# liuhx02/YourEditableAvatar

Hardware: AMD Instinct MI355X
Metric: rasterized fragments/sec (fwd+bwd) @500k Gaussians 1080p (higher is better)
Workload: dtype f32

## Files before the change

youreditableavatar_amd/csrc/tgs_api.hip:

```cpp
#include "tgs_device.hpp"
#include "../../include/tgs_raster.h"
#include "../../include/tgs_raster_testing.h"

#include <cstdarg>
#include <cstdio>
#include <cstring>

namespace tgs {
void launch_preprocess_fwd(hipStream_t, const FwdIn&, const CamParams&, const GeomState&, const ImgState&);
void launch_preprocess_fwd_batch(hipStream_t, const FwdIn&, const FwdViews&);
void launch_scan(hipStream_t, const GeomState&, const ImgState&, uint32_t nblocks, uint32_t T, uint32_t sort_cap, unsigned long long r_capacity,
                 uint32_t tile_bound, uint32_t heavy_bound, uint32_t mid_bound, Meta* host_meta, int light);
void launch_bin_count(hipStream_t, int P, const GeomState&, const ImgState&, uint32_t gx, uint32_t T);
void launch_scatter(hipStream_t, int P, const GeomState&, const ImgState&, const BinState&, uint32_t gx, uint32_t T);
void launch_tile_sort(hipStream_t, const GeomState&, const ImgState&, const BinState&, uint32_t gx, uint32_t T, uint64_t r_bound, const Meta* m,
                      uint32_t sort_cap, uint32_t tile_bound, uint32_t heavy_bound, uint32_t mid_bound);
void launch_render_fwd(hipStream_t, const ImgState&, const BinState&, int W, int H, uint32_t gx, uint32_t T, const Meta* m, const float* bg,
                       float* out_color, uint32_t tile_bound, uint32_t mid_bound, int light);
void launch_mark_visible(hipStream_t, int P, const float* means3D, const float* view, uint8_t* present);
void launch_render_bwd(hipStream_t, const ImgState&, const BinState&, int W, int H, uint32_t gx, uint32_t tiles, const float* bg, const float* dL_dpix,
                       bool deterministic, uint32_t mid_tiles, int light, uint32_t T);
void launch_preprocess_bwd(hipStream_t, const BwdIn&, const CamParams&, const GeomState&, const BinState&);
void launch_preprocess_bwd_batch(hipStream_t, const BwdIn&, const BatchViews&);
void launch_selftest_reduce36(hipStream_t, const float* in, float* out);
// ... 771 lines not shown

int tgs_backward_batch_range(void* stream, int P, int D, int M, int n_views, const tgs_view_t* views, const float* means3D, const float* shs,
                             const float* scales, float scale_modifier, const float* rotations, const float* cov3D_precomp, float* dL_dopacity,
                             float* dL_dmean3D, float* dL_dcov3D, float* dL_dsh, float* dL_dscale, float* dL_drot, int accumulate, int first, int count)
{
    return tgs_backward_batch_range_planes(stream, P, D, M, n_views, views, means3D, shs, scales, scale_modifier, rotations, cov3D_precomp, dL_dopacity, dL_dmean3D,
                                           dL_dcov3D, dL_dsh, dL_dscale, dL_drot, accumulate, first, count, 0);
}

int tgs_backward_batch_range_planes(void* stream, int P, int D, int M, int n_views, const tgs_view_t* views, const float* means3D, const float* shs,
                                    const float* scales, float scale_modifier, const float* rotations, const float* cov3D_precomp, float* dL_dopacity,
                                    float* dL_dmean3D, float* dL_dcov3D, float* dL_dsh, float* dL_dscale, float* dL_drot, int accumulate, int first, int count,
                                    int64_t dsh_plane_stride)
{
    hipStream_t st = (hipStream_t)stream;
    g_err[0] = 0;
    if (P == 0 || n_views == 0 || count == 0) return TGS_OK;
    if (P < 0 || n_views < 0 || !views) return fail(TGS_ERR_INVALID, "bad sizes");
    if (first < 0 || count < 0 || first % PRE_BLOCK != 0 || (long long)first + count > P || ((first + count) % PRE_BLOCK != 0 && first + count != P))
        return fail(TGS_ERR_INVALID, "Gaussian range [%d, %d + %d) must start and end on multiples of %d (or end at P = %d)", first, first, count, PRE_BLOCK, P);
    const Model m{P, D, M, means3D, shs, nullptr, nullptr, scales, scale_modifier, rotations, cov3D_precomp};
    const bool has_sh = m.has_sh(), has_sr = m.has_sr();
    if (int r = check_model(m, MODEL_BATCH_BACKWARD)) return r;
    if (!dL_dopacity || !dL_dmean3D || (has_sh && !dL_dsh) || (has_sr && (!dL_dscale || !dL_drot)) || (!has_sr && !dL_dcov3D))
        return fail(TGS_ERR_INVALID, "NULL required pointer");
    if (dsh_plane_stride != 0 && (!has_sh || M != 16 || dsh_plane_stride < 3 * (int64_t)P || dsh_plane_stride % 4 != 0 || ((uintptr_t)dL_dsh & 15u) != 0))
        return fail(TGS_ERR_INVALID, "level-major dL_dsh needs SH colours with M = 16, a plane stride >= 3 P that is a multiple of 4 floats, and a 16-byte aligned dL_dsh");
    BwdIn in = bwd_in(m);
    in.dL_dopacity = dL_dopacity; in.dL_dmean3D = dL_dmean3D; in.dL_dcov3D = has_sr ? nullptr : dL_dcov3D; in.dL_dsh = dL_dsh;
    in.dL_dscale = has_sr ? dL_dscale : nullptr; in.dL_drot = has_sr ? dL_drot : nullptr;
    in.block0 = first / PRE_BLOCK; in.nblocks = (int)n_blocks((size_t)count);
    in.dsh_plane = (long long)dsh_plane_stride;
    for (int v0 = 0; v0 < n_views; v0 += BATCH_VIEWS) {
        BatchViews bv;
        memset(&bv, 0, sizeof(bv));
        bv.n = n_views - v0 < BATCH_VIEWS ? n_views - v0 : BATCH_VIEWS;
        for (int k = 0; k < bv.n; k++) {
            const tgs_view_t& w = views[v0 + k];
            if (int r = check_view(w, v0 + k, VIEW_BATCH_BWD, has_sh)) return r;
            const ViewArgs v = view_args(w);
            const FrameBuffers fb = carve_frame(m.shape(), v, w.R, w.geom_buffer, w.binning_buffer, w.img_buffer);
            BatchView& o = bv.v[k];
            o.cam = v.cam(scale_modifier); o.g = fb.g; o.b = fb.b;
            o.meta = fb.s.meta; o.radii = w.radii; o.dL_dmean2D = w.dL_dmean2D; o.dL_dcolor = has_sh ? nullptr : w.dL_dcolor;
        }
        in.accumulate = (accumulate || v0 > 0) ? 1 : 0;
        if (int r = stage(st, TGS_STAGE_PREPROCESS_BWD, "preprocess_bwd_batch", 0, [&] { launch_preprocess_bwd_batch(st, in, bv); })) return r;
    }
    return TGS_OK;
}

int tgs_mark_visible(void* stream, int P, const float* means3D, const float* viewmatrix, const float* projmatrix, uint8_t* present)
{
    hipStream_t st = (hipStream_t)stream;
    g_err[0] = 0;
    (void)projmatrix;
    if (P == 0) return TGS_OK;
    if (P < 0 || !means3D || !viewmatrix || !present) return fail(TGS_ERR_INVALID, "bad arguments");
    launch_mark_visible(st, P, means3D, viewmatrix, present);
    hipError_t e = hipGetLastError();
    if (e != hipSuccess) return fail(TGS_ERR_HIP, "mark_visible: %s", hipGetErrorString(e));
    return TGS_OK;
}

int64_t tgs_state_field(void* stream, const char* field, int P, int width, int height, int64_t R, int has_sh, int has_scale_rot,
                        const void* geom_buffer, const void* binning_buffer, const void* img_buffer, void* dst, size_t dst_bytes)
{
    hipStream_t st = (hipStream_t)stream;
    g_err[0] = 0;
    const ViewArgs v{nullptr, width, height, nullptr, nullptr, nullptr, 0.f, 0.f};
    const size_t N = v.N(), T = v.T();
    const FrameBuffers fb = carve_frame(GeomShape{(size_t)P, has_sh != 0, has_scale_rot != 0}, v, R, geom_buffer, binning_buffer, img_buffer);
    const GeomState& g = fb.g; const ImgState& s = fb.s; const BinState& b = fb.b;
    const void* src = nullptr; size_t count = 0, esz = 4, stride = 0, rows = 0;
    if (!strcmp(field, "n_contrib")) { src = s.n_contrib; count = N; }
    else if (!strcmp(field, "final_T")) { src = s.final_T; count = N; }
    else if (!strcmp(field, "ranges")) { src = s.ranges; count = 2 * T; }
    else if (!strcmp(field, "means2D")) { src = g.pack; count = 2 * (size_t)P; esz = 8; stride = 64; rows = (size_t)P; }
    else if (!strcmp(field, "depths")) { src = g.depth; count = (size_t)P; }
    else if (!strcmp(field, "conic_opacity")) { src = (const char*)g.pack + 8; count = 4 * (size_t)P; esz = 16; stride = 64; rows = (size_t)P; }
    else if (!strcmp(field, "rgb")) { src = (const char*)g.pack + 24; count = 3 * (size_t)P; esz = 12; stride = 64; rows = (size_t)P; }
    else if (!strcmp(field, "tiles_touched")) { src = g.tiles_touched; count = (size_t)P; }
    else if (!strcmp(field, "tile_order")) { src = s.tile_order; count = T; }
    else if (!strcmp(field, "stamps")) { src = s.stamps; count = 8 * T; esz = 8; }
    else if (!strcmp(field, "block_masks")) { src = (const char*)b.recC + 4; count = (size_t)R; esz = 4; stride = 8; rows = (size_t)R; }
    else if (!strcmp(field, "quad_masks")) { src = b.qmask; count = (size_t)R; esz = 8; }
    else if (!strcmp(field, "point_list")) { src = b.keys; count = (size_t)R; esz = 4; stride = 8; rows = (size_t)R; }
    else return fail(TGS_ERR_INVALID, "unknown field %s", field);
    const size_t total = stride ? rows * esz : count * esz;
    if (dst_bytes < total) return fail(TGS_ERR_INVALID, "dst too small for %s", field);
    if (count == 0) return 0;
    if (stride) HIP_TRY(hipMemcpy2DAsync(dst, esz, src, stride, esz, rows, hipMemcpyDeviceToDevice, st));
    else HIP_TRY(hipMemcpyAsync(dst, src, total, hipMemcpyDeviceToDevice, st));
    return (int64_t)count;
}

}
```

youreditableavatar_amd/csrc/tgs_forward.hip:

```cpp
#include "tgs_device.hpp"

namespace tgs {

__device__ __forceinline__ float conic_min_on_edge(float dfix, float lo, float hi, float Pfix, float Pvar, float B, float mB_over_Pvar)
{
    const float t = fminf(hi, fmaxf(lo, dfix * mB_over_Pvar));
    return 0.5f * (Pfix * dfix * dfix + Pvar * t * t) + B * dfix * t;
}

__device__ __forceinline__ unsigned long long quadrant_mask(float2 xy, float4 co, uint32_t tx, uint32_t ty)
{
    const float o255 = 255.0f * co.w;
    if (o255 < 0.999f) return 0ull;
    const float tau = (fmaxf(__logf(o255), 0.f) + 0.01f) * 1.001f;
    const float A = co.x, B = co.y, Cc = co.z;
    const float det = A * Cc - B * B;
    if (!(det > 0.f && A > 0.f && Cc > 0.f)) return ~0ull;
    const float rA = __builtin_amdgcn_rcpf(A), K = 2.f * A * tau, sl = -B * rA;
    const float ox = xy.x - (float)(tx * TILE), y0 = (float)(ty * TILE) - xy.y;
    uint32_t keep[2] = {0u, 0u};
#pragma unroll
    for (int R = 0; R < 8; R++) {
        const float dy0 = y0 + (float)(2 * R), dy1 = y0 + (float)(2 * R + 1);
        const float d0 = fmaf(-det * dy0, dy0, K), d1 = fmaf(-det * dy1, dy1, K);
// ... 809 lines not shown
            for (uint32_t i = threadIdx.x; i < n; i += 1024) b.keys[td.y + i] = lk[i];
        }
    } else if (blockIdx.x < heavy_blocks + mid_blocks) {
        const uint32_t grp = threadIdx.x >> 8, tid = threadIdx.x & 255u;
        const uint32_t t = n_heavy + (blockIdx.x - heavy_blocks) * 4 + grp;
        if (n_heavy + (blockIdx.x - heavy_blocks) * 4 >= n_mid) return;
        uint32_t n = 0, start = 0, tile = 0;
        if (t < n_mid) { const uint4 td = s.tile_desc[t]; tile = td.x; start = td.y; n = td.z - td.y; }
        for (uint32_t i = tid; i < n; i += 256) b.tile_of[start + i] = tile;
        if (n > 1024u || n > sort_cap) n = 0;
        unsigned long long* seg = lk + grp * 1024;
        for (uint32_t i = tid; i < n; i += 256) seg[i] = b.keys[start + i];
        if (tid == 0) grp_npad[grp] = n < 2 ? 2u : next_pow2(n);
        __syncthreads();
        const uint32_t npad_wg = max(max(grp_npad[0], grp_npad[1]), max(grp_npad[2], grp_npad[3]));
        sort_tile_lds<256>(seg, tid, n, npad_wg);
        for (uint32_t i = tid; i < n; i += 256) b.keys[start + i] = seg[i];
    } else {
        const uint32_t t = n_mid + (blockIdx.x - heavy_blocks - mid_blocks) * 16 + wv;
        if (t >= n_nonempty) return;
        const uint4 td = s.tile_desc[t];
        const uint32_t n = td.z - td.y;
        for (uint32_t i = lane; i < n; i += 64) b.tile_of[td.y + i] = td.x;
        if (n < 2 || n > sort_cap || n > SORT_CHUNK) return;
        unsigned long long k0, k1;
        regs_load_chunk(b.keys + td.y, 0u, n, lane, k0, k1);
        if (n >= 2) {
            regs_sort128(k0, k1, lane);
            regs_store_chunk(b.keys + td.y, 0u, n, lane, k0, k1);
        }
    }
}

#ifndef TGS_FIN_E
#define TGS_FIN_E 2
#endif
constexpr int FIN_E = TGS_FIN_E;
__global__ __launch_bounds__(256) void k_finalize(const GeomState g, const ImgState s, const BinState b, uint32_t gx, uint32_t T)
{
    if (frame_rejected(s)) return;
    const uint32_t R = (uint32_t)s.meta->R;
    const uint32_t p0 = blockIdx.x * (256 * FIN_E) + threadIdx.x;
    if (p0 >= R) return;
    uint32_t id[FIN_E], tile[FIN_E];
#pragma unroll
    for (int e = 0; e < FIN_E; e++) {
        const uint32_t pc = min(p0 + e * 256, R - 1u);
        id[e] = (uint32_t)b.keys[pc];
        tile[e] = b.tile_of[pc];
    }
    float4 q0[FIN_E], q1[FIN_E], q2[FIN_E], q3[FIN_E];
#pragma unroll
    for (int e = 0; e < FIN_E; e++) {
        const float4* pk = g.pack + 4 * (size_t)id[e];
        q0[e] = pk[0]; q1[e] = pk[1]; q2[e] = pk[2]; q3[e] = pk[3];
    }
#pragma unroll
    for (int e = 0; e < FIN_E; e++) {
        const uint32_t p = p0 + e * 256;
        if (p < R) finalize_entry(q0[e], q1[e], q2[e], q3[e], p, tile[e], gx, b);
    }
}

__device__ __forceinline__ void fill_tile_background(const ImgState& s, uint32_t tile, uint32_t t, int W, int H, uint32_t gx,
                                                     const float* __restrict__ bg, float* __restrict__ out_color)
{
    const int px = (tile % gx) * TILE + (t & 15), py = (tile / gx) * TILE + (t >> 4);
    if (px < W && py < H) {
        const size_t pix_id = (size_t)W * py + px, N = (size_t)W * H;
        s.final_T[pix_id] = 1.0f;
        s.n_contrib[pix_id] = 0;
        out_color[pix_id] = bg[0]; out_color[N + pix_id] = bg[1]; out_color[2 * N + pix_id] = bg[2];
    }
}

constexpr int FQ_THREADS = 256;
#ifndef TGS_FQ_CH
#define TGS_FQ_CH 256
#endif
constexpr int FQ_CH = TGS_FQ_CH;
constexpr int FQ_EPT = FQ_CH / FQ_THREADS;
static_assert(FQ_CH % FQ_THREADS == 0 && FQ_CH >= LIGHT_MAX && FQ_CH <= 768, "whole entries per thread; a light tile is one round; slots are 10-bit in the block lists");
constexpr int FQ_NULL = FQ_CH;

__device__ __forceinline__ bool fwd_q_block_round(const float4* sA, const float4* sB, const float* sC, const uint2* sQ, unsigned short* list,
                                                  unsigned short (*ql)[QL_ROW_F], uint32_t cnt, int blk, int lane, uint32_t cbase, float pixfx, float pixfy,
                                                  float vone, const QuadMasks& qm, bool& done, float& T, float& C0, float& C1, float& C2, uint32_t& last_contributor)
{
    const int qd = lane >> 4, e = lane & 3;
    const uint32_t n = (uint32_t)__builtin_amdgcn_readfirstlane((int)build_own_list_q<FQ_CH>(list, sQ, cnt, blk, lane));
    const unsigned short* myq = &ql[qd][e];
#pragma unroll 1
    for (uint32_t c0 = 0; c0 < n; c0 += QCH_F) {
        const uint32_t nq = (uint32_t)__builtin_amdgcn_readfirstlane((int)build_chunk_quadrant_lists_128(ql, list, c0, n, lane, FQ_NULL));
        uint32_t jn = myq[0];
#pragma unroll 1
        for (uint32_t k = 0; k < nq; k += 4) {
            const uint32_t j = jn;
            jn = myq[k + 4];
            const float4 a = sA[j];
            const float4 bb = sB[j];
            const float cc = sC[j];
            const float dx = a.x - pixfx, dy = a.y - pixfy;
#if TGS_FAST_MATH
            const float power2 = pair_power2(a.z, a.w, bb.x, dx, dy);
            const float alpha = fminf(0.99f, bb.y * __builtin_amdgcn_exp2f(power2));
#else
            const float power2 = -0.5f * (a.z * dx * dx + bb.x * dy * dy) - a.w * dx * dy;
            const float alpha = fminf(0.99f, bb.y * expf(power2));
#endif
            const bool live = !done && !(power2 > 0.0f) && !(alpha < 1.0f / 255.0f);
            const float pown = live ? 1.f - alpha : 1.0f;
            float y, x, x3;
            fwd_chain4(pown, T, y, x, vone, qm);
            const bool fail = live && (x < 0.0001f);
            const bool upd = live && !fail;
            float cand = fail ? y : -1.0f;
            quad_max_bcast3(cand, x, x3);
            const float w = upd ? alpha * y : 0.f;
            C0 += bb.z * w; C1 += bb.w * w; C2 += cc * w;
            last_contributor = upd ? cbase + j : last_contributor;
            const bool stop = cand >= 0.0f;
            T = stop ? cand : x3;
            done = done || stop;
            if (__builtin_amdgcn_ballot_w64(!done) == 0) return true;
        }
    }
    return false;
}

__device__ __forceinline__ uint32_t fwd_q_block_store(const ImgState& s, float* __restrict__ out_color, int W, int H, int px, int py, bool inside, int lane,
                                                      float bg0, float bg1, float bg2, float T, float C0, float C1, float C2, uint32_t last_contributor)
{
    TGS_DPP_ADD(C0, 0xB1, 0xf); TGS_DPP_ADD(C0, 0x4E, 0xf);
    TGS_DPP_ADD(C1, 0xB1, 0xf); TGS_DPP_ADD(C1, 0x4E, 0xf);
    TGS_DPP_ADD(C2, 0xB1, 0xf); TGS_DPP_ADD(C2, 0x4E, 0xf);
    {
        uint32_t o = (uint32_t)__builtin_amdgcn_update_dpp(0, (int)last_contributor, 0xB1, 0xf, 0xf, false);
        last_contributor = max(last_contributor, o);
        o = (uint32_t)__builtin_amdgcn_update_dpp(0, (int)last_contributor, 0x4E, 0xf, 0xf, false);
        last_contributor = max(last_contributor, o);
    }
    if (inside && (lane & 3) == 0) {
        const size_t pix_id = (size_t)W * py + px, N = (size_t)W * H;
        s.final_T[pix_id] = T;
        s.n_contrib[pix_id] = last_contributor;
        out_color[pix_id] = C0 + T * bg0;
        out_color[N + pix_id] = C1 + T * bg1;
        out_color[2 * N + pix_id] = C2 + T * bg2;
    }
    return wave_max_u32(inside ? last_contributor : 0u);
}

__global__ __launch_bounds__(FQ_THREADS, 8) void k_render_fwd(const ImgState s, const BinState b, int W, int H, uint32_t gx,
                                                              const float* __restrict__ bg, float* __restrict__ out_color, uint32_t n_tiles, int light)
{
    __shared__ float4 sA[FQ_CH + 1];
    __shared__ float4 sB[FQ_CH + 1];
    __shared__ float sC[FQ_CH + 1];
    __shared__ uint2 sQ[FQ_CH];
    __shared__ __attribute__((aligned(16))) unsigned short lists[4][FQ_CH + 8];
    __shared__ __attribute__((aligned(16))) unsigned short qlists[4][4][QL_ROW_F];
    __shared__ uint32_t wave_alive[2][4];
    __shared__ uint32_t wave_qmax[4];
    const float bg0 = bg[0], bg1 = bg[1], bg2 = bg[2];
    const uint32_t hk = blockIdx.x >> 3, ht8 = (hk >> 2) * 8u + (blockIdx.x & 7u), quarter = hk & 3u;
    const uint4 tdh = s.tile_desc[min(ht8, n_tiles - 1u)];
    const uint4 ff = frame_counts(s);
    const uint32_t n_all = (ff.x & META_ERR_CAPACITY) ? 0u : ff.y;
    const uint32_t n_ne = light ? min(ff.w, n_all) : n_all;
    const uint32_t n_light = n_all - n_ne;
    const uint32_t heavy_wgs = 4u * ((n_ne + 7u) & ~7u);
    if (blockIdx.x == 0 && threadIdx.x == 0 && heavy_wgs + n_light > gridDim.x) atomicOr(&s.meta->error, META_ERR_TILE_BOUND);
    const int wv = threadIdx.x >> 6, lane = threadIdx.x & 63;
    const int qd = lane >> 4, pq = (lane >> 2) & 3;
    float vone = 1.0f;
    asm volatile("" : "+v"(vone));
    const QuadMasks qm = quad_masks();
    if (threadIdx.x == 0) { sA[FQ_NULL] = make_float4(0.f, 0.f, 0.f, 0.f); sB[FQ_NULL] = make_float4(0.f, 0.f, 0.f, 0.f); sC[FQ_NULL] = 0.f; }

    if (blockIdx.x >= heavy_wgs) {
        const uint32_t li = blockIdx.x - heavy_wgs;
        if (li >= n_light) {
            const uint32_t nfill = gridDim.x - heavy_wgs - n_light, j = li - n_light;
            for (uint32_t i = n_all + j; i < n_tiles; i += nfill)
                fill_tile_background(s, s.tile_desc[i].x, threadIdx.x, W, H, gx, bg, out_color);
            return;
        }
        const uint4 td = s.light_desc[li];
        const uint32_t tile = td.x, n = td.z - td.y;
        const uint32_t tx = tile % gx, ty = tile / gx;
        stamp(s, tile, 0);
        if (threadIdx.x < n) {
            const uint32_t pos = td.y + threadIdx.x;
            float4 va = b.recA[pos], vb = b.recB[pos];
            const float vc = b.recC[pos].x; const uint2 vq = b.qmask[pos];
#if TGS_FAST_MATH
            stage_conic_a(va); stage_conic_b(vb);
#endif
            sA[threadIdx.x] = va; sB[threadIdx.x] = vb; sC[threadIdx.x] = vc; sQ[threadIdx.x] = vq;
        }
        __syncthreads();
        uint32_t wq = 0;
#pragma unroll 1
        for (int bi = 0; bi < 4; bi++) {
            const int bx = (wv + bi) & 3, by = bi, blk = 4 * by + bx;
            const int px = tx * TILE + bx * 4 + (qd & 1) * 2 + (pq & 1);
            const int py = ty * TILE + by * 4 + (qd >> 1) * 2 + (pq >> 1);
            const bool inside = px < W && py < H;
            bool done = !inside;
            if (__builtin_amdgcn_ballot_w64(!done) == 0) continue;
            float T = 1.0f, C0 = 0.f, C1 = 0.f, C2 = 0.f;
            uint32_t last_contributor = 0;
            fwd_q_block_round(sA, sB, sC, sQ, lists[wv], qlists[wv], n, blk, lane, 1u, (float)px, (float)py, vone, qm, done, T, C0, C1, C2, last_contributor);
            wq = max(wq, fwd_q_block_store(s, out_color, W, H, px, py, inside, lane, bg0, bg1, bg2, T, C0, C1, C2, last_contributor));
        }
        if (lane == 0) wave_qmax[wv] = wq;
        __syncthreads();
        if (threadIdx.x == 0) {
            const uint32_t q = max(max(wave_qmax[0], wave_qmax[1]), max(wave_qmax[2], wave_qmax[3]));
            reinterpret_cast<uint32_t*>(&s.light_desc[li])[3] = q;
            reinterpret_cast<uint32_t*>(&s.tile_desc[n_ne + li])[3] = q;
        }
        stamp(s, tile, 1);
        return;
    }
    if (ht8 >= n_ne) return;
    const uint32_t tile = tdh.x;
    const uint32_t tx = tile % gx, ty = tile / gx;
    const int bx = 2 * (int)(quarter & 1u) + (wv & 1), by = 2 * (int)(quarter >> 1) + (wv >> 1), blk = 4 * by + bx;
    const int px = tx * TILE + bx * 4 + (qd & 1) * 2 + (pq & 1);
    const int py = ty * TILE + by * 4 + (qd >> 1) * 2 + (pq >> 1);
    const bool inside = px < W && py < H;
    const float pixfx = (float)px, pixfy = (float)py;
    const uint2 rg = make_uint2(tdh.y, tdh.z);
    set_wave_priority(rg.y - rg.x);
    if (quarter == 0) stamp(s, tile, 0);
    bool done = !inside;
    float T = 1.0f, C0 = 0.f, C1 = 0.f, C2 = 0.f;
    uint32_t last_contributor = 0;
    float4 ra[FQ_EPT], rb[FQ_EPT]; float rc[FQ_EPT]; uint2 rq[FQ_EPT];
#pragma unroll
    for (int i = 0; i < FQ_EPT; i++) { ra[i] = make_float4(0.f, 0.f, 0.f, 0.f); rb[i] = ra[i]; rc[i] = 0.f; rq[i] = make_uint2(0u, 0u); }
#define TGS_FQ_FETCH(BASE) { _Pragma("unroll") for (int i = 0; i < FQ_EPT; i++) { const uint32_t pos = (BASE) + (uint32_t)(i * FQ_THREADS) + threadIdx.x; \
        if (pos < rg.y) { ra[i] = b.recA[pos]; rb[i] = b.recB[pos]; rc[i] = b.recC[pos].x; rq[i] = b.qmask[pos]; } } }
    TGS_FQ_FETCH(rg.x)
    bool wave_live = __builtin_amdgcn_ballot_w64(!done) != 0;
    int round = 0;
    for (uint32_t base = rg.x; base < rg.y; base += FQ_CH, round++) {
        if (lane == 0) wave_alive[round & 1][wv] = wave_live ? 1u : 0u;
        __syncthreads();
        {
            const uint4 f = *reinterpret_cast<const uint4*>(wave_alive[round & 1]);
            if ((f.x | f.y | f.z | f.w) == 0u) break;
        }
        const uint32_t cnt = min((uint32_t)FQ_CH, rg.y - base);
#pragma unroll
        for (int i = 0; i < FQ_EPT; i++) {
            const uint32_t h = (uint32_t)(i * FQ_THREADS) + threadIdx.x;
            if (h < cnt) {
                float4 va = ra[i], vb = rb[i];
#if TGS_FAST_MATH
                stage_conic_a(va); stage_conic_b(vb);
#endif
                sA[h] = va; sB[h] = vb; sC[h] = rc[i]; sQ[h] = rq[i];
            }
        }
        __syncthreads();
        if (base + FQ_CH < rg.y) TGS_FQ_FETCH(base + FQ_CH)
        if (wave_live && fwd_q_block_round(sA, sB, sC, sQ, lists[wv], qlists[wv], cnt, blk, lane, base - rg.x + 1, pixfx, pixfy, vone, qm, done, T, C0, C1, C2, last_contributor))
            wave_live = false;
    }
#undef TGS_FQ_FETCH
    const uint32_t m = fwd_q_block_store(s, out_color, W, H, px, py, inside, lane, bg0, bg1, bg2, T, C0, C1, C2, last_contributor);
    if (lane == 0) wave_qmax[wv] = m;
    __syncthreads();
    if (threadIdx.x == 0) {
        const uint32_t q = max(max(wave_qmax[0], wave_qmax[1]), max(wave_qmax[2], wave_qmax[3]));
        atomicMax(reinterpret_cast<uint32_t*>(&s.tile_desc[ht8]) + 3, q);
        if (ht8 >= ff.w) atomicMax(reinterpret_cast<uint32_t*>(&s.light_desc[ht8 - ff.w]) + 3, q);
    }
    stamp_max(s, tile, 1);
}

__global__ __launch_bounds__(256) void k_mark_visible(int P, const float* __restrict__ means3D, const float* __restrict__ view, uint8_t* present)
{
    const int idx = blockIdx.x * 256 + threadIdx.x;
    if (idx >= P) return;
    const float mx = means3D[3 * (size_t)idx], my = means3D[3 * (size_t)idx + 1], mz = means3D[3 * (size_t)idx + 2];
    const float z = view[2] * mx + view[6] * my + view[10] * mz + view[14];
    present[idx] = !(z <= 0.2f);
}

void launch_preprocess_fwd(hipStream_t st, const FwdIn& in, const CamParams& cam, const GeomState& g, const ImgState& s)
{
    const dim3 grid((unsigned)n_blocks(in.P)), blk(PRE_BLOCK);
    const bool sh = in.colors_precomp == nullptr, sr = in.cov3D_precomp == nullptr;
    FwdView vw;
    vw.cam = cam; vw.g = g; vw.s = s; vw.radii = in.radii;
    if (sh && sr) hipLaunchKernelGGL((k_preprocess_fwd<true, true>), grid, blk, 0, st, in, vw);
    else if (sh) hipLaunchKernelGGL((k_preprocess_fwd<true, false>), grid, blk, 0, st, in, vw);
    else if (sr) hipLaunchKernelGGL((k_preprocess_fwd<false, true>), grid, blk, 0, st, in, vw);
    else hipLaunchKernelGGL((k_preprocess_fwd<false, false>), grid, blk, 0, st, in, vw);
}
void launch_preprocess_fwd_batch(hipStream_t st, const FwdIn& in, const FwdViews& views)
{
    const dim3 grid((unsigned)n_blocks(in.P)), blk(PRE_BLOCK);
    const bool sh = in.colors_precomp == nullptr, sr = in.cov3D_precomp == nullptr;
    if (views.n == 2) {
        if (sh && sr) hipLaunchKernelGGL((k_preprocess_fwd_pair<true, true>), grid, blk, 0, st, in, views.v[0], views.v[1]);
        else if (sh) hipLaunchKernelGGL((k_preprocess_fwd_pair<true, false>), grid, blk, 0, st, in, views.v[0], views.v[1]);
        else if (sr) hipLaunchKernelGGL((k_preprocess_fwd_pair<false, true>), grid, blk, 0, st, in, views.v[0], views.v[1]);
        else hipLaunchKernelGGL((k_preprocess_fwd_pair<false, false>), grid, blk, 0, st, in, views.v[0], views.v[1]);
        return;
    }
    if (sh && sr) hipLaunchKernelGGL((k_preprocess_fwd_batch<true, true>), grid, blk, 0, st, in, views);
    else if (sh) hipLaunchKernelGGL((k_preprocess_fwd_batch<true, false>), grid, blk, 0, st, in, views);
    else if (sr) hipLaunchKernelGGL((k_preprocess_fwd_batch<false, true>), grid, blk, 0, st, in, views);
    else hipLaunchKernelGGL((k_preprocess_fwd_batch<false, false>), grid, blk, 0, st, in, views);
}
void launch_scan(hipStream_t st, const GeomState& g, const ImgState& s, uint32_t nblocks, uint32_t T, uint32_t sort_cap, unsigned long long r_capacity,
                 uint32_t tile_bound, uint32_t heavy_bound, uint32_t mid_bound, Meta* host_meta, int light)
{
    hipLaunchKernelGGL(k_scan, dim3(1u + (T + SCAN_THREADS - 1) / SCAN_THREADS), dim3(SCAN_THREADS), 0, st, g, s, nblocks, T, sort_cap, r_capacity, tile_bound, heavy_bound, mid_bound,
                       host_meta, light);
}
void bin_shape(int P, uint32_t T, uint32_t& nchunks, uint32_t& chunk, uint32_t& band, size_t& lds)
{
    static const int bin_wgs = [] {
        const char* e = getenv("TGS_BIN_WGS");
        const int v = e ? atoi(e) : BIN_WGS_MAX;
        return v < 1 ? 1 : (v > BIN_WGS_MAX ? BIN_WGS_MAX : v);
    }();
    const uint32_t per = ((uint32_t)P + (uint32_t)bin_wgs - 1) / (uint32_t)bin_wgs;
    chunk = (per + BIN_THREADS - 1) / BIN_THREADS * BIN_THREADS;
    if (chunk == 0) chunk = BIN_THREADS;
    nchunks = ((uint32_t)P + chunk - 1) / chunk;
    band = T < BIN_LDS_TILES ? T : BIN_LDS_TILES;
    lds = (size_t)band * sizeof(uint32_t);
}
void launch_bin_count(hipStream_t st, int P, const GeomState& g, const ImgState& s, uint32_t gx, uint32_t T)
{
    uint32_t nchunks, chunk, band; size_t lds;
    bin_shape(P, T, nchunks, chunk, band, lds);
    if (lds > 32 * 1024) (void)hipFuncSetAttribute((const void*)k_bin_count, hipFuncAttributeMaxDynamicSharedMemorySize, (int)lds);
    hipLaunchKernelGGL(k_bin_count, dim3(nchunks), dim3(BIN_THREADS), lds, st, P, chunk, g, s, gx, T, band);
    hipLaunchKernelGGL(k_bin_colscan, dim3((T + WAVE - 1) / WAVE), dim3(64 * COL_WAVES), 0, st, s, T, nchunks);
}
void launch_scatter(hipStream_t st, int P, const GeomState& g, const ImgState& s, const BinState& b, uint32_t gx, uint32_t T)
{
    uint32_t nchunks, chunk, band; size_t lds;
    bin_shape(P, T, nchunks, chunk, band, lds);
    if (lds > 32 * 1024) (void)hipFuncSetAttribute((const void*)k_scatter, hipFuncAttributeMaxDynamicSharedMemorySize, (int)lds);
    hipLaunchKernelGGL(k_scatter, dim3(nchunks), dim3(BIN_THREADS), lds, st, P, chunk, g, s, b, gx, T, band);
}
static uint32_t host_next_pow2(uint32_t n) { uint32_t p = 1; while (p < n) p <<= 1; return p; }
// ... 46 lines not shown
```

youreditableavatar_amd/diff_gaussian_rasterization/_C.py:

```python
from __future__ import annotations

import ctypes as C
import os
from typing import Optional, Tuple

import torch

from .. import build as _build

_LIB_PATH = os.environ.get("TGS_LIBRARY") or _build.LIB


ABI_VERSION = 3


def _load() -> C.CDLL:
    if "TGS_LIBRARY" not in os.environ:
        try:
            _build.build_native()
        except Exception as e:
            what = "is older than its sources" if os.path.exists(_LIB_PATH) else "is missing"
            raise ImportError(f"libtgs_raster.so {what} and could not be rebuilt ({e}); run "
                              f"`python -c 'import __graft_entry__ as g; g.build()'` on a ROCm machine") from e
    lib = C.CDLL(_LIB_PATH, mode=C.RTLD_GLOBAL)
# ... 280 lines not shown
    arr = (C.c_void_p * max(1, len(stream_handles)))(*stream_handles)
    _lib.tgs_set_render_streams(arr, len(stream_handles))


def backward_render_views(stream_handles, P, views, n_views, opt: Optional[_OptionsT] = None) -> None:
    arr = (C.c_void_p * len(stream_handles))(*stream_handles)
    r = _lib.tgs_backward_render_views_opt(C.byref(opt) if opt is not None else None, arr, len(stream_handles), int(P), int(n_views),
                                           views if isinstance(views, C.c_void_p) else C.cast(views, C.c_void_p))
    if r < 0:
        raise _err(int(r))


def backward_batch_raw(stream, P, D, M, views, n_views, means3D, shs, scales, scale_modifier, rotations, dL_dopacity, dL_dmean3D, dL_dsh, dL_dscale,
                       dL_drot, accumulate, first: int = 0, count: Optional[int] = None, dsh_plane_stride: int = 0) -> None:
    args = (stream, int(P), int(D), int(M), int(n_views), views if isinstance(views, C.c_void_p) else C.cast(views, C.c_void_p), means3D, shs,
            scales, float(scale_modifier),
            rotations, None, dL_dopacity, dL_dmean3D, None, dL_dsh if shs else None, dL_dscale, dL_drot, 1 if accumulate else 0,
            int(first), int(P - first if count is None else count))
    r = _lib.tgs_backward_batch_range_planes(*args, int(dsh_plane_stride)) if dsh_plane_stride else _lib.tgs_backward_batch_range(*args)
    if r < 0:
        raise _err(int(r))


def rasterize_gaussians_backward_render(background, dL_dout_color, R, binningBuffer, imageBuffer, P, tile_bound: int = 0,
                                        deterministic: Optional[bool] = None) -> None:
    dev = _require_gpu(dL_dout_color)
    H, W = int(dL_dout_color.size(1)), int(dL_dout_color.size(2))
    with torch.cuda.device(dev):
        bg, dL = _dev_f32(background, dev, "background"), _dev_f32(dL_dout_color, dev, "dL_dout_color")
        opt = options(tile_bound=tile_bound, deterministic=deterministic)
        r = _lib.tgs_backward_render_opt(C.byref(opt), torch.cuda.current_stream(dev).cuda_stream, int(P), int(R), _p(bg), W, H, binningBuffer.data_ptr(),
                                         imageBuffer.data_ptr(), _p(dL))
    if r < 0:
        raise _err(int(r))


def rasterize_gaussians_backward_batch(views, means3D, sh, degree, scales, rotations, scale_modifier, cov3D_precomp, into, accumulate=True):
    dev = _require_gpu(means3D)
    P = int(means3D.size(0))
    M = int(sh.size(1)) if (sh is not None and sh.dim() > 1 and sh.size(0) != 0) else 0
    has_sh = M > 0
    outs = []
    if P == 0 or not views:
        return outs
    with torch.cuda.device(dev):
        t = dict(means=_dev_f32(means3D, dev, "means3D"), sh=_dev_f32(sh, dev, "sh") if has_sh else None, scales=_dev_f32(scales, dev, "scales"),
                 rots=_dev_f32(rotations, dev, "rotations"), cov=_dev_f32(cov3D_precomp, dev, "cov3D_precomp"))
        has_sr = t["scales"] is not None
        arr = (_ViewT * len(views))()
        keep = []
        for i, v in enumerate(views):
            vm, pm, cp = _dev_f32(v["viewmatrix"], dev, "viewmatrix"), _dev_f32(v["projmatrix"], dev, "projmatrix"), _dev_f32(v["campos"], dev, "campos")
            radii = v["radii"].contiguous()
            g2d = torch.empty((P, 3), dtype=torch.float32, device=dev)
            gcol = None if has_sh else torch.empty((P, 3), dtype=torch.float32, device=dev)
            keep += [vm, pm, cp, radii]
            a = arr[i]
            a.width, a.height, a.tan_fovx, a.tan_fovy = int(v["image_width"]), int(v["image_height"]), float(v["tanfovx"]), float(v["tanfovy"])
            a.viewmatrix, a.projmatrix, a.campos, a.radii = vm.data_ptr(), pm.data_ptr(), cp.data_ptr(), radii.data_ptr()
            a.geom_buffer, a.binning_buffer, a.img_buffer, a.R = v["geom"].data_ptr(), v["binning"].data_ptr(), v["img"].data_ptr(), int(v["R"])
            a.dL_dmean2D, a.dL_dcolor = g2d.data_ptr(), (gcol.data_ptr() if gcol is not None else None)
            outs.append((g2d, gcol))

        def dst(name, shape):
            g = into.get(name)
            if g is None:
                raise RuntimeError(f"rasterize_gaussians_backward_batch: no gradient buffer for {name}")
            if g.dtype != torch.float32 or g.device != dev or not g.is_contiguous() or tuple(g.shape) != shape:
                raise RuntimeError(f"gradient buffer for {name} must be a contiguous fp32 tensor of shape {shape} on {dev}")
            return g.data_ptr()

        r = _lib.tgs_backward_batch(torch.cuda.current_stream(dev).cuda_stream, P, int(degree), M, len(views), C.cast(arr, C.c_void_p), _p(t["means"]),
                                    _p(t["sh"]), _p(t["scales"]), float(scale_modifier), _p(t["rots"]), _p(t["cov"]), dst("opacities", (P, 1)),
                                    dst("means3D", (P, 3)), None if has_sr else dst("cov3D_precomp", (P, 6)), dst("sh", (P, M, 3)) if has_sh else None,
                                    dst("scales", (P, 3)) if has_sr else None, dst("rotations", (P, 4)) if has_sr else None, 1 if accumulate else 0)
        del keep
    if r < 0:
        raise _err(int(r))
    return outs


_FIELD_DTYPES = {"n_contrib": torch.int32, "final_T": torch.float32, "ranges": torch.int32, "point_list": torch.int32, "block_masks": torch.int32,
                 "means2D": torch.float32, "depths": torch.float32, "conic_opacity": torch.float32, "rgb": torch.float32,
                 "tiles_touched": torch.int32, "tile_order": torch.int32, "stamps": torch.int64, "quad_masks": torch.int64}


def state_field(name: str, P: int, width: int, height: int, R: int, has_sh: bool, has_scale_rot: bool,
                geomBuffer, binningBuffer, imageBuffer) -> torch.Tensor:
    dev = geomBuffer.device
    T = ((width + 15) // 16) * ((height + 15) // 16)
    count = {"n_contrib": width * height, "final_T": width * height, "ranges": 2 * T, "point_list": R, "block_masks": R, "quad_masks": R, "means2D": 2 * P,
             "depths": P, "conic_opacity": 4 * P, "rgb": 3 * P, "tiles_touched": P, "tile_order": T, "stamps": 8 * T}[name]
    out = torch.empty((count,), dtype=_FIELD_DTYPES[name], device=dev)
    with torch.cuda.device(dev):
        r = _lib.tgs_state_field(torch.cuda.current_stream(dev).cuda_stream, name.encode(), P, width, height, int(R),
                                 int(has_sh), int(has_scale_rot), geomBuffer.data_ptr(), binningBuffer.data_ptr(),
                                 imageBuffer.data_ptr(), out.data_ptr(), out.numel() * out.element_size())
    if r < 0:
        raise _err(int(r))
    return out


rasterize_gaussians = _ext.rasterize_gaussians
rasterize_gaussians_backward = _ext.rasterize_gaussians_backward
mark_visible = _ext.mark_visible
```

Baseline: 951,200.

## Compact per-quarter gaussian lists in heavy-tile forward render before staging

The heavy-tile forward render path now scans each tile's block masks, selects only the entries whose mask touches the block's quarter, and gathers just those records into shared memory in FQ_CH-sized rounds. This is done with ballot-based stream compaction that is double-buffered against the render of the previous round. Quad-mask staging shrinks to the relevant 32-bit half, and chunk boundaries are split wherever selected entries cross an original round. The goal is to cut global loads and per-round work spent on gaussians that never affect this quarter. The cost is extra barriers, shared memory and a scan pass over the masks. A tile_desc debug field is also exposed.

```diff
diff --git a/youreditableavatar_amd/csrc/tgs_api.hip b/youreditableavatar_amd/csrc/tgs_api.hip
--- a/youreditableavatar_amd/csrc/tgs_api.hip
+++ b/youreditableavatar_amd/csrc/tgs_api.hip
@@ -877,6 +877,7 @@
     else if (!strcmp(field, "rgb")) { src = (const char*)g.pack + 24; count = 3 * (size_t)P; esz = 12; stride = 64; rows = (size_t)P; }
     else if (!strcmp(field, "tiles_touched")) { src = g.tiles_touched; count = (size_t)P; }
     else if (!strcmp(field, "tile_order")) { src = s.tile_order; count = T; }
+    else if (!strcmp(field, "tile_desc")) { src = s.tile_desc; count = 4 * T; }
     else if (!strcmp(field, "stamps")) { src = s.stamps; count = 8 * T; esz = 8; }
     else if (!strcmp(field, "block_masks")) { src = (const char*)b.recC + 4; count = (size_t)R; esz = 4; stride = 8; rows = (size_t)R; }
     else if (!strcmp(field, "quad_masks")) { src = b.qmask; count = (size_t)R; esz = 8; }
diff --git a/youreditableavatar_amd/csrc/tgs_forward.hip b/youreditableavatar_amd/csrc/tgs_forward.hip
--- a/youreditableavatar_amd/csrc/tgs_forward.hip
+++ b/youreditableavatar_amd/csrc/tgs_forward.hip
@@ -915,17 +915,44 @@
 constexpr int FQ_EPT = FQ_CH / FQ_THREADS;
 static_assert(FQ_CH % FQ_THREADS == 0 && FQ_CH >= LIGHT_MAX && FQ_CH <= 768, "whole entries per thread; a light tile is one round; slots are 10-bit in the block lists");
 constexpr int FQ_NULL = FQ_CH;
-
+#ifndef TGS_FQ_WIN_EPT
+#define TGS_FQ_WIN_EPT 4
+#endif
+#ifndef TGS_FQ_PRE
+#define TGS_FQ_PRE 1
+#endif
+constexpr int FQ_WIN_EPT = TGS_FQ_WIN_EPT;
+constexpr int FQ_PRE = TGS_FQ_PRE;
+constexpr int FQ_PRE_N = FQ_PRE > 0 ? FQ_PRE : 1;
+static_assert(FQ_WIN_EPT >= 1 && FQ_WIN_EPT <= 4 && FQ_PRE >= 0 && FQ_PRE <= FQ_WIN_EPT, "the selection window: one to four masks per thread");
+
+__device__ __forceinline__ uint32_t fwd_q_chunk_end(const unsigned short* list, const uint32_t* pos1, uint32_t c0, uint32_t cend, int lane)
+{
+    const uint32_t r0 = (pos1[list[c0] & 1023u] - 1u) / (uint32_t)FQ_CH;
+#pragma unroll
+    for (int h = 0; h < QCH_F / 64; h++) {
+        const uint32_t i = c0 + 64u * h + lane;
+        const bool brk = i < cend && (pos1[list[min(i, cend - 1u)] & 1023u] - 1u) / (uint32_t)FQ_CH != r0;
+        const unsigned long long bal = __builtin_amdgcn_ballot_w64(brk);
+        if (bal) return c0 + 64u * h + (uint32_t)__builtin_ctzll(bal);
+    }
+    return cend;
+}
+
+template <bool QUARTER>
 __device__ __forceinline__ bool fwd_q_block_round(const float4* sA, const float4* sB, const float* sC, const uint2* sQ, unsigned short* list,
                                                   unsigned short (*ql)[QL_ROW_F], uint32_t cnt, int blk, int lane, uint32_t cbase, float pixfx, float pixfy,
-                                                  float vone, const QuadMasks& qm, bool& done, float& T, float& C0, float& C1, float& C2, uint32_t& last_contributor)
+                                                  float vone, const QuadMasks& qm, bool& done, float& T, float& C0, float& C1, float& C2, uint32_t& last_contributor,
+                                                  const uint32_t* pos1 = nullptr)
 {
     const int qd = lane >> 4, e = lane & 3;
     const uint32_t n = (uint32_t)__builtin_amdgcn_readfirstlane((int)build_own_list_q<FQ_CH>(list, sQ, cnt, blk, lane));
     const unsigned short* myq = &ql[qd][e];
 #pragma unroll 1
-    for (uint32_t c0 = 0; c0 < n; c0 += QCH_F) {
-        const uint32_t nq = (uint32_t)__builtin_amdgcn_readfirstlane((int)build_chunk_quadrant_lists_128(ql, list, c0, n, lane, FQ_NULL));
+    for (uint32_t c0 = 0, cend; c0 < n; c0 = cend) {
+        cend = min(c0 + (uint32_t)QCH_F, n);
+        if (QUARTER) cend = (uint32_t)__builtin_amdgcn_readfirstlane((int)fwd_q_chunk_end(list, pos1, c0, cend, lane));
+        const uint32_t nq = (uint32_t)__builtin_amdgcn_readfirstlane((int)build_chunk_quadrant_lists_128(ql, list, c0, cend, lane, FQ_NULL));
         uint32_t jn = myq[0];
 #pragma unroll 1
         for (uint32_t k = 0; k < nq; k += 4) {
@@ -985,6 +1012,69 @@
     return wave_max_u32(inside ? last_contributor : 0u);
 }
 
+constexpr uint32_t FQ_SLOT_TAG = 0x80000000u;
+template <int N>
+__device__ __forceinline__ void fq_fetch_masks(const BinState& b, uint32_t rgx, uint32_t n_list, uint32_t from, uint32_t (&mk)[N])
+{
+#pragma unroll
+    for (int i = 0; i < N; i++) {
+        const uint32_t off = from + (uint32_t)(i * FQ_THREADS) + threadIdx.x;
+        mk[i] = off < n_list ? __float_as_uint(b.recC[rgx + off].y) : 0u;
+    }
+}
+struct FqSel { uint32_t np, scan, par; bool over; };
+template <int N>
+__device__ __forceinline__ bool fq_select_window(FqSel& sel, uint32_t n_list, uint32_t qbits, const uint32_t (&mk)[N], uint32_t* pos1,
+                                                 uint32_t (*cnts)[FQ_WIN_EPT][4], uint32_t* sel_next, int wv, int lane)
+{
+    static_assert(N <= FQ_WIN_EPT, "the count exchange holds FQ_WIN_EPT stretches");
+    uint32_t rk[N];
+#pragma unroll
+    for (int i = 0; i < N; i++) {
+        const unsigned long long bal = __builtin_amdgcn_ballot_w64((mk[i] & qbits) != 0u);
+        rk[i] = __builtin_amdgcn_mbcnt_hi((uint32_t)(bal >> 32), __builtin_amdgcn_mbcnt_lo((uint32_t)bal, 0u));
+        if (lane == 0) cnts[sel.par][i][wv] = (uint32_t)__builtin_popcountll(bal);
+    }
+    __syncthreads();
+    uint32_t run = sel.np;
+#pragma unroll
+    for (int i = 0; i < N; i++) {
+        const uint4 c = *reinterpret_cast<const uint4*>(cnts[sel.par][i]);
+        const uint32_t before = run + (wv > 0 ? c.x : 0u) + (wv > 1 ? c.y : 0u) + (wv > 2 ? c.z : 0u);
+        const uint32_t r = (uint32_t)__builtin_amdgcn_readfirstlane((int)before) + rk[i];
+        const uint32_t off = sel.scan + (uint32_t)(i * FQ_THREADS) + threadIdx.x;
+        if ((mk[i] & qbits) != 0u) {
+            if (r < (uint32_t)FQ_CH) pos1[r] = off + 1u;
+            else if (r == (uint32_t)FQ_CH) *sel_next = off;
+        }
+        run = (uint32_t)__builtin_amdgcn_readfirstlane((int)(run + c.x + c.y + c.z + c.w));
+    }
+    sel.par ^= 1u;
+    if (run > (uint32_t)FQ_CH) { sel.np = (uint32_t)FQ_CH; sel.over = true; return true; }
+    sel.np = run;
+    sel.scan += (uint32_t)(N * FQ_THREADS);
+    return run == (uint32_t)FQ_CH || sel.scan >= n_list;
+}
+template <int PRE>
+__device__ __forceinline__ uint32_t fq_select_round(FqSel& sel, const BinState& b, uint32_t rgx, uint32_t n_list, uint32_t qbits, const uint32_t (&mk0)[PRE > 0 ? PRE : 1],
+                                                    uint32_t* pos1, uint32_t (*cnts)[FQ_WIN_EPT][4], uint32_t* sel_next, int wv, int lane)
+{
+    sel.np = 0;
+    sel.over = false;
+    if (PRE > 0) {
+        constexpr int REST = FQ_WIN_EPT - PRE > 0 ? FQ_WIN_EPT - PRE : 1;
+        uint32_t m[REST];
+        fq_fetch_masks<REST>(b, rgx, n_list, sel.scan + (uint32_t)(PRE * FQ_THREADS), m);
+        if (fq_select_window<(PRE > 0 ? PRE : 1)>(sel, n_list, qbits, mk0, pos1, cnts, sel_next, wv, lane)) return sel.np;
+        if (fq_select_window<REST>(sel, n_list, qbits, m, pos1, cnts, sel_next, wv, lane)) return sel.np;
+    }
+    for (;;) {
+        uint32_t m[FQ_WIN_EPT];
+        fq_fetch_masks<FQ_WIN_EPT>(b, rgx, n_list, sel.scan, m);
+        if (fq_select_window<FQ_WIN_EPT>(sel, n_list, qbits, m, pos1, cnts, sel_next, wv, lane)) return sel.np;
+    }
+}
+
 __global__ __launch_bounds__(FQ_THREADS, 8) void k_render_fwd(const ImgState s, const BinState b, int W, int H, uint32_t gx,
                                                               const float* __restrict__ bg, float* __restrict__ out_color, uint32_t n_tiles, int light)
 {
@@ -996,6 +1086,9 @@
     __shared__ __attribute__((aligned(16))) unsigned short qlists[4][4][QL_ROW_F];
     __shared__ uint32_t wave_alive[2][4];
     __shared__ uint32_t wave_qmax[4];
+    __shared__ __attribute__((aligned(16))) uint32_t sPos[2][FQ_CH];
+    __shared__ __attribute__((aligned(16))) uint32_t sel_cnt[2][FQ_WIN_EPT][4];
+    __shared__ uint32_t sel_next;
     const float bg0 = bg[0], bg1 = bg[1], bg2 = bg[2];
     const uint32_t hk = blockIdx.x >> 3, ht8 = (hk >> 2) * 8u + (blockIdx.x & 7u), quarter = hk & 3u;
     const uint4 tdh = s.tile_desc[min(ht8, n_tiles - 1u)];
@@ -1045,7 +1138,7 @@
             if (__builtin_amdgcn_ballot_w64(!done) == 0) continue;
             float T = 1.0f, C0 = 0.f, C1 = 0.f, C2 = 0.f;
             uint32_t last_contributor = 0;
-            fwd_q_block_round(sA, sB, sC, sQ, lists[wv], qlists[wv], n, blk, lane, 1u, (float)px, (float)py, vone, qm, done, T, C0, C1, C2, last_contributor);
+            fwd_q_block_round<false>(sA, sB, sC, sQ, lists[wv], qlists[wv], n, blk, lane, 1u, (float)px, (float)py, vone, qm, done, T, C0, C1, C2, last_contributor);
             wq = max(wq, fwd_q_block_store(s, out_color, W, H, px, py, inside, lane, bg0, bg1, bg2, T, C0, C1, C2, last_contributor));
         }
         if (lane == 0) wave_qmax[wv] = wq;
@@ -1072,22 +1165,30 @@
     bool done = !inside;
     float T = 1.0f, C0 = 0.f, C1 = 0.f, C2 = 0.f;
     uint32_t last_contributor = 0;
-    float4 ra[FQ_EPT], rb[FQ_EPT]; float rc[FQ_EPT]; uint2 rq[FQ_EPT];
-#pragma unroll
-    for (int i = 0; i < FQ_EPT; i++) { ra[i] = make_float4(0.f, 0.f, 0.f, 0.f); rb[i] = ra[i]; rc[i] = 0.f; rq[i] = make_uint2(0u, 0u); }
-#define TGS_FQ_FETCH(BASE) { _Pragma("unroll") for (int i = 0; i < FQ_EPT; i++) { const uint32_t pos = (BASE) + (uint32_t)(i * FQ_THREADS) + threadIdx.x; \
-        if (pos < rg.y) { ra[i] = b.recA[pos]; rb[i] = b.recB[pos]; rc[i] = b.recC[pos].x; rq[i] = b.qmask[pos]; } } }
-    TGS_FQ_FETCH(rg.x)
+    const uint32_t n_list = rg.y - rg.x;
+    const uint32_t qbits = 0x33u << (2u * (quarter & 1u) + 8u * (quarter >> 1));
+    const uint32_t* qhalf = reinterpret_cast<const uint32_t*>(b.qmask) + (quarter >> 1);
+    uint32_t* sQh = reinterpret_cast<uint32_t*>(sQ) + (quarter >> 1);
+    float4 ra[FQ_EPT], rb[FQ_EPT]; float rc[FQ_EPT]; uint32_t rq[FQ_EPT]; uint32_t mk[FQ_PRE_N];
+#pragma unroll
+    for (int i = 0; i < FQ_EPT; i++) { ra[i] = make_float4(0.f, 0.f, 0.f, 0.f); rb[i] = ra[i]; rc[i] = 0.f; rq[i] = 0u; }
+#define TGS_FQ_GATHER(PL, CNT) { _Pragma("unroll") for (int i = 0; i < FQ_EPT; i++) { const uint32_t h = (uint32_t)(i * FQ_THREADS) + threadIdx.x; \
+        if (h < (CNT)) { const uint32_t pos = rg.x + (PL)[h] - 1u; ra[i] = b.recA[pos]; rb[i] = b.recB[pos]; rc[i] = b.recC[pos].x; rq[i] = qhalf[2 * (size_t)pos]; } } }
+    FqSel sel{0u, 0u, 0u, false};
+    if (FQ_PRE > 0) fq_fetch_masks<FQ_PRE_N>(b, rg.x, n_list, sel.scan, mk);
+    uint32_t cnt = fq_select_round<FQ_PRE>(sel, b, rg.x, n_list, qbits, mk, sPos[0], sel_cnt, &sel_next, wv, lane);
+    __syncthreads();
+    if (sel.over) sel.scan = (uint32_t)__builtin_amdgcn_readfirstlane((int)sel_next);
+    TGS_FQ_GATHER(sPos[0], cnt)
+    if (FQ_PRE > 0 && sel.scan < n_list) fq_fetch_masks<FQ_PRE_N>(b, rg.x, n_list, sel.scan, mk);
     bool wave_live = __builtin_amdgcn_ballot_w64(!done) != 0;
-    int round = 0;
-    for (uint32_t base = rg.x; base < rg.y; base += FQ_CH, round++) {
+    for (int round = 0; cnt > 0; round++) {
         if (lane == 0) wave_alive[round & 1][wv] = wave_live ? 1u : 0u;
         __syncthreads();
         {
             const uint4 f = *reinterpret_cast<const uint4*>(wave_alive[round & 1]);
             if ((f.x | f.y | f.z | f.w) == 0u) break;
         }
-        const uint32_t cnt = min((uint32_t)FQ_CH, rg.y - base);
 #pragma unroll
         for (int i = 0; i < FQ_EPT; i++) {
             const uint32_t h = (uint32_t)(i * FQ_THREADS) + threadIdx.x;
@@ -1096,15 +1197,27 @@
 #if TGS_FAST_MATH
                 stage_conic_a(va); stage_conic_b(vb);
 #endif
-                sA[h] = va; sB[h] = vb; sC[h] = rc[i]; sQ[h] = rq[i];
+                sA[h] = va; sB[h] = vb; sC[h] = rc[i]; sQh[2 * h] = rq[i];
             }
         }
-        __syncthreads();
-        if (base + FQ_CH < rg.y) TGS_FQ_FETCH(base + FQ_CH)
-        if (wave_live && fwd_q_block_round(sA, sB, sC, sQ, lists[wv], qlists[wv], cnt, blk, lane, base - rg.x + 1, pixfx, pixfy, vone, qm, done, T, C0, C1, C2, last_contributor))
-            wave_live = false;
-    }
-#undef TGS_FQ_FETCH
+        const uint32_t* pos1 = sPos[round & 1];
+        uint32_t* pos1_next = sPos[(round + 1) & 1];
+        uint32_t cnt_next = 0;
+        sel.over = false;
+        if (sel.scan < n_list) cnt_next = fq_select_round<FQ_PRE>(sel, b, rg.x, n_list, qbits, mk, pos1_next, sel_cnt, &sel_next, wv, lane);
+        __syncthreads();
+        if (sel.over) sel.scan = (uint32_t)__builtin_amdgcn_readfirstlane((int)sel_next);
+        TGS_FQ_GATHER(pos1_next, cnt_next)
+        if (FQ_PRE > 0 && sel.scan < n_list) fq_fetch_masks<FQ_PRE_N>(b, rg.x, n_list, sel.scan, mk);
+        if (wave_live) {
+            uint32_t lc = 0;
+            if (fwd_q_block_round<true>(sA, sB, sC, sQ, lists[wv], qlists[wv], cnt, blk, lane, FQ_SLOT_TAG, pixfx, pixfy, vone, qm, done, T, C0, C1, C2, lc, pos1))
+                wave_live = false;
+            if (lc) last_contributor = pos1[lc & 1023u];
+        }
+        cnt = cnt_next;
+    }
+#undef TGS_FQ_GATHER
     const uint32_t m = fwd_q_block_store(s, out_color, W, H, px, py, inside, lane, bg0, bg1, bg2, T, C0, C1, C2, last_contributor);
     if (lane == 0) wave_qmax[wv] = m;
     __syncthreads();
diff --git a/youreditableavatar_amd/diff_gaussian_rasterization/_C.py b/youreditableavatar_amd/diff_gaussian_rasterization/_C.py
--- a/youreditableavatar_amd/diff_gaussian_rasterization/_C.py
+++ b/youreditableavatar_amd/diff_gaussian_rasterization/_C.py
@@ -386,7 +386,7 @@
 
 _FIELD_DTYPES = {"n_contrib": torch.int32, "final_T": torch.float32, "ranges": torch.int32, "point_list": torch.int32, "block_masks": torch.int32,
                  "means2D": torch.float32, "depths": torch.float32, "conic_opacity": torch.float32, "rgb": torch.float32,
-                 "tiles_touched": torch.int32, "tile_order": torch.int32, "stamps": torch.int64, "quad_masks": torch.int64}
+                 "tiles_touched": torch.int32, "tile_order": torch.int32, "tile_desc": torch.int32, "stamps": torch.int64, "quad_masks": torch.int64}
 
 
 def state_field(name: str, P: int, width: int, height: int, R: int, has_sh: bool, has_scale_rot: bool,
@@ -394,7 +394,7 @@
     dev = geomBuffer.device
     T = ((width + 15) // 16) * ((height + 15) // 16)
     count = {"n_contrib": width * height, "final_T": width * height, "ranges": 2 * T, "point_list": R, "block_masks": R, "quad_masks": R, "means2D": 2 * P,
-             "depths": P, "conic_opacity": 4 * P, "rgb": 3 * P, "tiles_touched": P, "tile_order": T, "stamps": 8 * T}[name]
+             "depths": P, "conic_opacity": 4 * P, "rgb": 3 * P, "tiles_touched": P, "tile_order": T, "tile_desc": 4 * T, "stamps": 8 * T}[name]
     out = torch.empty((count,), dtype=_FIELD_DTYPES[name], device=dev)
     with torch.cuda.device(dev):
         r = _lib.tgs_state_field(torch.cuda.current_stream(dev).cuda_stream, name.encode(), P, width, height, int(R),
```

Result: slower. 941,300 (-1.0%).
